# jeun-990806/pim-jpeg-decoder

Measured on AMD Instinct MI355X. Metric: MPixels/sec JPEG->RGB (bit-exact BMP), higher is better.
Workload: dtype int16/int32 (integer IDCT), u8 out

## Files before the change

### pim-jpeg-decoder_amd/csrc/pjd_device_common.h

```cpp
#pragma once
#include <hip/hip_runtime.h>
#include <stdint.h>

#include "pjd_internal.h"

static __constant__ uint8_t c_zz[64] = {
     0,  1,  8, 16,  9,  2,  3, 10, 17, 24, 32, 25, 18, 11,  4,  5,
    12, 19, 26, 33, 40, 48, 41, 34, 27, 20, 13,  6,  7, 14, 21, 28,
    35, 42, 49, 56, 57, 50, 43, 36, 29, 22, 15, 23, 30, 37, 44, 51,
    38, 59, 52, 45, 38, 31, 39, 46, 53, 60, 61, 54, 47, 55, 62, 63
};

__device__ __forceinline__ int pjd_mul_i24(int a, int k)
{
    int r;
    asm("v_mul_i32_i24 %0, %1, %2" : "=v"(r) : "s"(k), "v"(a));
    return r;
}

__device__ __forceinline__ void pjd_idct8(int x0, int x1, int x2, int x3, int x4, int x5, int x6, int x7, int *o)
{
    const int g0 = pjd_mul_i24(x0, 181) >> 5, g1 = pjd_mul_i24(x4, 181) >> 5;
    const int g2 = pjd_mul_i24(x2, 59) >> 3,  g3 = pjd_mul_i24(x6, 49) >> 4;
    const int g4 = pjd_mul_i24(x5, 71) >> 4,  g5 = pjd_mul_i24(x1, 251) >> 5;
    const int g6 = pjd_mul_i24(x7, 25) >> 4,  g7 = pjd_mul_i24(x3, 213) >> 5;
    const int f4 = g4 - g7, f5 = g5 + g6, f6 = g5 - g6, f7 = g4 + g7;
    const int e2 = g2 - g3, e3 = g2 + g3, e5 = f5 - f7, e7 = f5 + f7, e8 = f4 + f6;
    const int d2 = pjd_mul_i24(e2, 181) >> 7, d4 = pjd_mul_i24(f4, 277) >> 8, d5 = pjd_mul_i24(e5, 181) >> 7;
    const int d6 = pjd_mul_i24(f6, 669) >> 8, d8 = pjd_mul_i24(e8, 49) >> 6;
    const int c0 = g0 + g1, c1 = g0 - g1, c2 = d2 - e3, c4 = d4 + d8;
    const int c5 = d5 + e7, c6 = d6 - d8, c8 = c5 - c6;
    const int b0 = c0 + e3, b1 = c1 + c2, b2 = c1 - c2, b3 = c0 - e3, b4 = c4 - c8, b6 = c6 - e7;
    o[0] = (b0 + e7) >> 4; o[1] = (b1 + b6) >> 4; o[2] = (b2 + c8) >> 4; o[3] = (b3 + b4) >> 4;
    o[4] = (b3 - b4) >> 4; o[5] = (b2 - c8) >> 4; o[6] = (b1 - b6) >> 4; o[7] = (b0 - e7) >> 4;
}

__device__ __forceinline__ int pjd_clamp255(int v)
{
    int r;
    asm("v_med3_i32 %0, %1, 0, %2" : "=v"(r) : "v"(v), "s"(255));
    return r;
}

__device__ __forceinline__ void pjd_ycc_to_rgb(int y, int cb, int cr, int &r, int &g, int &b)
{
    r = pjd_clamp255(y + (__mul24(5880414, cr) >> 22) + 128);
    g = pjd_clamp255(y - (__mul24(1442840, cb) >> 22) - (__mul24(2994733, cr) >> 22) + 128);
    b = pjd_clamp255(y + (__mul24(7432306, cb) >> 22) + 128);
}

__device__ __forceinline__ uint32_t pjd_mul_u24(uint32_t a, uint32_t b)
{
    uint32_t r;
    asm("v_mul_u32_u24 %0, %1, %2" : "=v"(r) : "v"(a), "v"(b));
    return r;
}
__device__ __forceinline__ uint32_t pjd_mad_u24(uint32_t a, uint32_t b, uint32_t c)
{
    uint32_t r;
    asm("v_mad_u32_u24 %0, %1, %2, %3" : "=v"(r) : "v"(a), "v"(b), "v"(c));
    return r;
}

__device__ __forceinline__ int pjd_dequant(int coef, unsigned q) { return (int)(int16_t)__mul24(coef, (int)q); }
```

### pim-jpeg-decoder_amd/csrc/pjd_k_backend.hip

```cpp
#include <cstdlib>

#include "pjd_device_common.h"
#include "pjd_kernels.h"

#define TILE_STRIDE 72

__global__ __launch_bounds__(128) void pjd_k_dpu_payload(const uint32_t *__restrict__ meta_all, int16_t *__restrict__ mcus_all)
{
    __shared__ __attribute__((aligned(16))) int16_t tile[12][TILE_STRIDE];
    const int dpu = blockIdx.x / 25, blk = blockIdx.x % 25;
    const uint32_t *m = meta_all + (size_t)dpu * 276;
    int16_t *base = mcus_all + (size_t)dpu * 19200 + blk * 768;
    const int tid = threadIdx.x;
    const int ncomp = (int)m[4];
    const int V = (int)(m[5] & 255), H = (int)(m[6] & 255);

    if (tid < 96) {
        const int du = tid >> 3, r = tid & 7, comp = du >> 2;
        const int4 raw = *reinterpret_cast<const int4 *>(base + du * 64 + r * 8);
        const int16_t *rv = reinterpret_cast<const int16_t *>(&raw);
        int x[8], o[8];
#pragma unroll
        for (int j = 0; j < 8; j++) x[j] = rv[j];
        if (comp < ncomp) {
// ... 261 lines not shown
            if (Y >= height) continue;
            const int16_t *yp = &tile[d0 + lrow + (px0 >> 3)][yoff + (px0 & 7)];
            const uint2 yraw = *reinterpret_cast<const uint2 *>(yp);
            const int y0 = (int16_t)(yraw.x & 0xffff), y1 = (int16_t)(yraw.x >> 16), y2 = (int16_t)(yraw.y & 0xffff), y3 = (int16_t)(yraw.y >> 16);
            const uint32_t q = cy * 8 + (px0 >> hs_log);
            int cf[4], cg[4], cl[4];
            const int n_chroma = hs == 2 ? 2 : 4;
            uint2 cbw = make_uint2(0, 0), crw = make_uint2(0, 0);
            if (nc > 1) { if (hs == 2) cbw.x = *reinterpret_cast<const uint32_t *>(&tile[d0 + nl][q]); else cbw = *reinterpret_cast<const uint2 *>(&tile[d0 + nl][q]); }
            if (nc > 2) { if (hs == 2) crw.x = *reinterpret_cast<const uint32_t *>(&tile[d0 + nl + 1][q]); else crw = *reinterpret_cast<const uint2 *>(&tile[d0 + nl + 1][q]); }
#pragma unroll
            for (int j = 0; j < 4; j++) {
                if (j < n_chroma) {
                    const uint32_t bw = j < 2 ? cbw.x : cbw.y, rw = j < 2 ? crw.x : crw.y;
                    const int cbv = (j & 1) ? (int)(int16_t)(bw >> 16) : (int)(int16_t)(bw & 0xffff);
                    const int crv = (j & 1) ? (int)(int16_t)(rw >> 16) : (int)(int16_t)(rw & 0xffff);
                    const int rC = (__mul24(5880414, crv) >> 22) + 128, bC = (__mul24(7432306, cbv) >> 22) + 128;
                    cg[j] = 128 - (__mul24(1442840, cbv) >> 22) - (__mul24(2994733, crv) >> 22);
                    cf[j] = bmp ? bC : rC;
                    cl[j] = bmp ? rC : bC;
                }
            }
            const int s1 = hs == 2 ? 0 : 1, s2 = hs == 2 ? 1 : 2, s3 = hs == 2 ? 1 : 3;
            const int cf1 = s1 ? cf[1] : cf[0], cg1 = s1 ? cg[1] : cg[0], cl1 = s1 ? cl[1] : cl[0];
            const int cf2 = s2 == 2 ? cf[2] : cf[1], cg2 = s2 == 2 ? cg[2] : cg[1], cl2 = s2 == 2 ? cl[2] : cl[1];
            const int cf3 = s3 == 3 ? cf[3] : cf[1], cg3 = s3 == 3 ? cg[3] : cg[1], cl3 = s3 == 3 ? cl[3] : cl[1];
            const uint32_t f0 = pjd_clamp255(y0 + cf[0]), g0 = pjd_clamp255(y0 + cg[0]), l0 = pjd_clamp255(y0 + cl[0]);
            const uint32_t f1 = pjd_clamp255(y1 + cf1), g1 = pjd_clamp255(y1 + cg1), l1 = pjd_clamp255(y1 + cl1);
            const uint32_t f2 = pjd_clamp255(y2 + cf2), g2 = pjd_clamp255(y2 + cg2), l2 = pjd_clamp255(y2 + cl2);
            const uint32_t f3 = pjd_clamp255(y3 + cf3), g3 = pjd_clamp255(y3 + cg3), l3 = pjd_clamp255(y3 + cl3);
            if (PLANAR) {
                const size_t plane = (size_t)stride * height;
                uint8_t *o = out + (size_t)Y * stride + X;
                if (X + 4 <= width) {
                    reinterpret_cast<PjdPx4 *>(o)->a = f0 | (f1 << 8) | (f2 << 16) | (f3 << 24);
                    reinterpret_cast<PjdPx4 *>(o + plane)->a = g0 | (g1 << 8) | (g2 << 16) | (g3 << 24);
                    reinterpret_cast<PjdPx4 *>(o + 2 * plane)->a = l0 | (l1 << 8) | (l2 << 16) | (l3 << 24);
                } else {
                    o[0] = (uint8_t)f0; o[plane] = (uint8_t)g0; o[2 * plane] = (uint8_t)l0;
                    if (X + 1 < width) { o[1] = (uint8_t)f1; o[plane + 1] = (uint8_t)g1; o[2 * plane + 1] = (uint8_t)l1; }
                    if (X + 2 < width) { o[2] = (uint8_t)f2; o[plane + 2] = (uint8_t)g2; o[2 * plane + 2] = (uint8_t)l2; }
                }
                continue;
            }
            uint8_t *o = bmp ? out + 26 + (size_t)(height - 1 - Y) * stride + X * 3
                             : out + (size_t)Y * stride + X * 3;
            if (X + 4 <= width) {
                Px12 v;
                v.a = f0 | (g0 << 8) | (l0 << 16) | (f1 << 24);
                v.b = g1 | (l1 << 8) | (f2 << 16) | (g2 << 24);
                v.c = l2 | (f3 << 8) | (g3 << 16) | (l3 << 24);
                *reinterpret_cast<Px12 *>(o) = v;
            } else {
                o[0] = (uint8_t)f0; o[1] = (uint8_t)g0; o[2] = (uint8_t)l0;
                if (X + 1 < width) { o[3] = (uint8_t)f1; o[4] = (uint8_t)g1; o[5] = (uint8_t)l1; }
                if (X + 2 < width) { o[6] = (uint8_t)f2; o[7] = (uint8_t)g2; o[8] = (uint8_t)l2; }
            }
        }
    }
}

struct __attribute__((packed)) PjdPx12 { uint32_t a, b, c; };

template <int HS, int VS, bool BMP, bool PLANAR = false>
__device__ __forceinline__ void pjd_colour_store(const int16_t (*tile)[TILE_STRIDE], const uint32_t *mcu_xy, uint8_t *out,
                                                 uint32_t width, uint32_t height, uint32_t stride, uint32_t ncomp,
                                                 uint32_t n_mcu, uint32_t tid, size_t plane = 0)
{
    static_assert(!(BMP && PLANAR), "a BMP file image is interleaved");
    constexpr uint32_t MW = 8 * HS, MH = 8 * VS, NL = HS * VS;
    constexpr uint32_t CG_LOG = HS == 2 ? 2 : 1;
    constexpr int NCH = 4 / HS;
    const uint32_t dus = NL + ncomp - 1;
    const uint32_t per_row = n_mcu << CG_LOG;
    const uint32_t lane = tid & 63, wv = tid >> 6;
    for (uint32_t rg = wv; rg < 8; rg += PJD_IDCT_THREADS / 64) {
        for (uint32_t idx = lane; idx < per_row; idx += 64) {
            const uint32_t ml = idx >> CG_LOG, px0 = (idx & ((1u << CG_LOG) - 1)) * 4;
            const uint32_t xy = mcu_xy[ml];
            const uint32_t X = __umul24(xy & 0xffffu, MW) + px0, Y0 = __umul24(xy >> 16, MH) + rg * VS;
            if (X >= width || Y0 >= height) continue;
            const uint32_t d0 = __umul24(ml, dus);
            int cf[NCH], cg[NCH], cl[NCH];
            {
                const uint32_t q = rg * 8 + px0 / HS;
                uint32_t cbw[2] = {0, 0}, crw[2] = {0, 0};
                if (ncomp > 1) {
                    if (HS == 2) cbw[0] = *reinterpret_cast<const uint32_t *>(&tile[d0 + NL][q]);
                    else { const uint2 t = *reinterpret_cast<const uint2 *>(&tile[d0 + NL][q]); cbw[0] = t.x; cbw[1] = t.y; }
                }
                if (ncomp > 2) {
                    if (HS == 2) crw[0] = *reinterpret_cast<const uint32_t *>(&tile[d0 + NL + 1][q]);
                    else { const uint2 t = *reinterpret_cast<const uint2 *>(&tile[d0 + NL + 1][q]); crw[0] = t.x; crw[1] = t.y; }
                }
#pragma unroll
                for (int j = 0; j < NCH; j++) {
                    const uint32_t bw = cbw[j >> 1], rw = crw[j >> 1];
                    const int cbv = (j & 1) ? (int)bw >> 16 : (int)(int16_t)(bw & 0xffff);
                    const int crv = (j & 1) ? (int)rw >> 16 : (int)(int16_t)(rw & 0xffff);
                    const int rC = (__mul24(5880414, crv) >> 22) + 128, bC = (__mul24(7432306, cbv) >> 22) + 128;
                    cg[j] = 128 - (__mul24(1442840, cbv) >> 22) - (__mul24(2994733, crv) >> 22);
                    cf[j] = BMP ? bC : rC;
                    cl[j] = BMP ? rC : bC;
                }
            }
#pragma unroll
            for (int v = 0; v < VS; v++) {
                const uint32_t Y = Y0 + v;
                if (Y >= height) break;
                const uint32_t py = rg * VS + v;
                const int16_t *yp = &tile[d0 + (py >> 3) * HS + (px0 >> 3)][(py & 7) * 8 + (px0 & 7)];
                const uint2 yraw = *reinterpret_cast<const uint2 *>(yp);
                const int y0 = (int16_t)(yraw.x & 0xffff), y1 = (int)yraw.x >> 16, y2 = (int16_t)(yraw.y & 0xffff), y3 = (int)yraw.y >> 16;
                constexpr int s1 = HS == 2 ? 0 : 1, s2 = HS == 2 ? 1 : 2, s3 = HS == 2 ? 1 : 3;
                const uint32_t f0 = pjd_clamp255(y0 + cf[0]), g0 = pjd_clamp255(y0 + cg[0]), l0 = pjd_clamp255(y0 + cl[0]);
                const uint32_t f1 = pjd_clamp255(y1 + cf[s1]), g1 = pjd_clamp255(y1 + cg[s1]), l1 = pjd_clamp255(y1 + cl[s1]);
                const uint32_t f2 = pjd_clamp255(y2 + cf[s2]), g2 = pjd_clamp255(y2 + cg[s2]), l2 = pjd_clamp255(y2 + cl[s2]);
                const uint32_t f3 = pjd_clamp255(y3 + cf[s3]), g3 = pjd_clamp255(y3 + cg[s3]), l3 = pjd_clamp255(y3 + cl[s3]);
                if (PLANAR) {
                    uint8_t *o = out + (size_t)Y * stride + X;
                    if (X + 4 <= width) {
                        reinterpret_cast<PjdPx4 *>(o)->a = f0 | (f1 << 8) | (f2 << 16) | (f3 << 24);
                        reinterpret_cast<PjdPx4 *>(o + plane)->a = g0 | (g1 << 8) | (g2 << 16) | (g3 << 24);
                        reinterpret_cast<PjdPx4 *>(o + 2 * plane)->a = l0 | (l1 << 8) | (l2 << 16) | (l3 << 24);
                    } else {
                        o[0] = (uint8_t)f0; o[plane] = (uint8_t)g0; o[2 * plane] = (uint8_t)l0;
                        if (X + 1 < width) { o[1] = (uint8_t)f1; o[plane + 1] = (uint8_t)g1; o[2 * plane + 1] = (uint8_t)l1; }
                        if (X + 2 < width) { o[2] = (uint8_t)f2; o[plane + 2] = (uint8_t)g2; o[2 * plane + 2] = (uint8_t)l2; }
                    }
                    continue;
                }
                uint8_t *o = BMP ? out + 26 + (size_t)(height - 1 - Y) * stride + X * 3 : out + (size_t)Y * stride + X * 3;
                if (X + 4 <= width) {
                    PjdPx12 px;
                    px.a = f0 | (g0 << 8) | (l0 << 16) | (f1 << 24);
                    px.b = g1 | (l1 << 8) | (f2 << 16) | (g2 << 24);
                    px.c = l2 | (f3 << 8) | (g3 << 16) | (l3 << 24);
                    *reinterpret_cast<PjdPx12 *>(o) = px;
                } else {
                    o[0] = (uint8_t)f0; o[1] = (uint8_t)g0; o[2] = (uint8_t)l0;
                    if (X + 1 < width) { o[3] = (uint8_t)f1; o[4] = (uint8_t)g1; o[5] = (uint8_t)l1; }
                    if (X + 2 < width) { o[6] = (uint8_t)f2; o[7] = (uint8_t)g2; o[8] = (uint8_t)l2; }
                }
            }
        }
    }
}

__device__ __forceinline__ void pjd_bmp_header(uint8_t *out, uint32_t width, uint32_t height, uint32_t stride, uint32_t tid)
{
    if (tid >= 26) return;
    const uint32_t size = 26 + height * stride;
    uint8_t hb = 0;
    switch (tid) {
        case 0: hb = 'B'; break;  case 1: hb = 'M'; break;
        case 2: hb = size & 255; break; case 3: hb = (size >> 8) & 255; break;
        case 4: hb = (size >> 16) & 255; break; case 5: hb = (size >> 24) & 255; break;
        case 10: hb = 0x1A; break; case 14: hb = 12; break;
        case 18: hb = width & 255; break; case 19: hb = (width >> 8) & 255; break;
        case 20: hb = height & 255; break; case 21: hb = (height >> 8) & 255; break;
        case 22: hb = 1; break; case 24: hb = 24; break;
        default: hb = 0;
    }
    out[tid] = hb;
}

template <int HS, int VS, bool BMP, int S, bool PLANAR = false>
__device__ __forceinline__ void pjd_colour_store_scaled(const int16_t (*tile)[TILE_STRIDE], const uint32_t *mcu_xy, uint8_t *out,
                                                        uint32_t width, uint32_t height, uint32_t stride, uint32_t ncomp,
                                                        uint32_t n_mcu, uint32_t tid)
{
    static_assert(!(BMP && PLANAR), "a BMP file image is interleaved");
    constexpr uint32_t MW = 8 * HS, MH = 8 * VS, NL = HS * VS;
    constexpr uint32_t CG_LOG = HS == 2 ? 2 : 1;
    constexpr uint32_t S_LOG = S == 2 ? 1 : (S == 4 ? 2 : 3);
    constexpr uint32_t BR_LOG = (VS == 2 ? 4 : 3) - S_LOG;
    constexpr int NCH = 4 / HS;
    constexpr int NO = S < 4 ? 4 / S : 1;
    constexpr int PX_LOG = S < 4 ? S_LOG : 2;
    static_assert(MH % S == 0 && S % VS == 0, "a box lies inside one MCU and covers whole chroma rows");
    const uint32_t dus = NL + ncomp - 1;
    const uint32_t tasks = n_mcu << (CG_LOG + BR_LOG);
    const uint32_t sh = (height + S - 1) >> S_LOG;
    for (uint32_t t = tid; t < tasks; t += PJD_IDCT_THREADS) {
        const uint32_t ml = t >> (CG_LOG + BR_LOG), j = (t >> CG_LOG) & ((1u << BR_LOG) - 1), px0 = (t & ((1u << CG_LOG) - 1)) * 4;
        const uint32_t xy = mcu_xy[ml];
        const uint32_t X = __umul24(xy & 0xffffu, MW) + px0, Yb = __umul24(xy >> 16, MH) + j * S;
// ... 117 lines not shown

template <bool SCALED, bool PLANAR = false>
__device__ __forceinline__ void pjd_colour_dispatch(const int16_t (*tile)[TILE_STRIDE], const uint32_t *mcu_xy, const PjdDevBatch &B,
                                                    const PjdDevImage &im, const PjdDevIdctWg &wg, uint32_t tid)
{
    if (SCALED && (im.flags & PJD_IF_SCALE_MASK)) { pjd_colour_dispatch_scaled<PLANAR>(tile, mcu_xy, B, im, wg, tid); return; }
    uint8_t *out = B.out + im.out_off;
    const uint32_t width = im.width, height = im.height, stride = im.out_stride, nc = im.ncomp, n = wg.n_mcu;
    if (PLANAR) {
        const size_t plane = (size_t)stride * height;
        switch ((im.hs - 1) | ((im.vs - 1) << 1)) {
            case 0: pjd_colour_store<1, 1, false, true>(tile, mcu_xy, out, width, height, stride, nc, n, tid, plane); break;
            case 1: pjd_colour_store<2, 1, false, true>(tile, mcu_xy, out, width, height, stride, nc, n, tid, plane); break;
            case 2: pjd_colour_store<1, 2, false, true>(tile, mcu_xy, out, width, height, stride, nc, n, tid, plane); break;
            default: pjd_colour_store<2, 2, false, true>(tile, mcu_xy, out, width, height, stride, nc, n, tid, plane); break;
        }
        return;
    }
    const bool bmp = (im.flags & PJD_IF_BMP) != 0;
    if (bmp && wg.first_mcu == 0) pjd_bmp_header(out, width, height, stride, tid);
    const uint32_t mode = (im.hs - 1) | ((im.vs - 1) << 1) | (bmp ? 4u : 0u);
    switch (mode) {
        case 0: pjd_colour_store<1, 1, false>(tile, mcu_xy, out, width, height, stride, nc, n, tid); break;
        case 1: pjd_colour_store<2, 1, false>(tile, mcu_xy, out, width, height, stride, nc, n, tid); break;
        case 2: pjd_colour_store<1, 2, false>(tile, mcu_xy, out, width, height, stride, nc, n, tid); break;
        case 3: pjd_colour_store<2, 2, false>(tile, mcu_xy, out, width, height, stride, nc, n, tid); break;
        case 4: pjd_colour_store<1, 1, true>(tile, mcu_xy, out, width, height, stride, nc, n, tid); break;
        case 5: pjd_colour_store<2, 1, true>(tile, mcu_xy, out, width, height, stride, nc, n, tid); break;
        case 6: pjd_colour_store<1, 2, true>(tile, mcu_xy, out, width, height, stride, nc, n, tid); break;
        default: pjd_colour_store<2, 2, true>(tile, mcu_xy, out, width, height, stride, nc, n, tid); break;
    }
}

template <bool SCALED>
__global__ __launch_bounds__(PJD_IDCT_THREADS) void pjd_k_idct_colour(PjdDevBatch B, const PjdDevIdctWg *__restrict__ wgs, const uint64_t *__restrict__ dense_base)
{
#define PJD_DENSE_PLANAR false
#include "pjd_k_idct_dense_body.h"
#undef PJD_DENSE_PLANAR
}

template <bool SCALED>
__global__ __launch_bounds__(PJD_IDCT_THREADS) void pjd_k_idct_colour_planar(PjdDevBatch B, const PjdDevIdctWg *__restrict__ wgs, const uint64_t *__restrict__ dense_base)
{
#define PJD_DENSE_PLANAR true
#include "pjd_k_idct_dense_body.h"
#undef PJD_DENSE_PLANAR
}


#define PJD_DPP_STEP(OP, v, ctrl, rmask)                                                               \
    do { const uint32_t t_ = (uint32_t)__builtin_amdgcn_update_dpp(0, (int)(v), ctrl, rmask, 0xf, false); v = OP(v, t_); } while (0)
__device__ __forceinline__ uint32_t pjd_op_add(uint32_t a, uint32_t b) { return a + b; }
__device__ __forceinline__ uint32_t pjd_op_max(uint32_t a, uint32_t b) { return a > b ? a : b; }
__device__ __forceinline__ uint32_t pjd_op_pkadd(uint32_t a, uint32_t b)
{
    typedef unsigned short u16x2 __attribute__((ext_vector_type(2)));
    return __builtin_bit_cast(uint32_t, (u16x2)(__builtin_bit_cast(u16x2, a) + __builtin_bit_cast(u16x2, b)));
}
__device__ __forceinline__ uint32_t pjd_op_pksub(uint32_t a, uint32_t b)
{
    typedef unsigned short u16x2 __attribute__((ext_vector_type(2)));
    return __builtin_bit_cast(uint32_t, (u16x2)(__builtin_bit_cast(u16x2, a) - __builtin_bit_cast(u16x2, b)));
}
#define PJD_WAVE_SCAN(OP, v)                                                                           \
    do {                                                                                                \
        PJD_DPP_STEP(OP, v, 0x111, 0xf); PJD_DPP_STEP(OP, v, 0x112, 0xf); PJD_DPP_STEP(OP, v, 0x114, 0xf);  \
        PJD_DPP_STEP(OP, v, 0x118, 0xf); PJD_DPP_STEP(OP, v, 0x142, 0xa); PJD_DPP_STEP(OP, v, 0x143, 0xc);  \
    } while (0)
__device__ __forceinline__ uint32_t pjd_wave_prev(uint32_t v)
{
    const uint32_t r = (uint32_t)__builtin_amdgcn_update_dpp(0, (int)v, 0x138 , 0xf, 0xf, false);
    return r;
}

__device__ __forceinline__ void pjd_tile_put(uint32_t tile_lds, uint32_t u, uint32_t pos, uint32_t v)
{
    const uint32_t a = pjd_mad_u24(u, TILE_STRIDE * 2u, tile_lds + 2u * pos);
    *reinterpret_cast<__attribute__((address_space(3))) int16_t *>(a) = (int16_t)v;
}

template <bool SCALED, bool PLANAR = false>
__device__ __forceinline__ void pjd_idct_range(const PjdDevBatch &B, uint32_t iwg, int16_t (*tile)[TILE_STRIDE], uint32_t (*qz)[64], uint32_t *mcu_xy,
                                               uint8_t *comp_of, uint32_t *wagg, uint32_t *ltab)
{
    const PjdDevIdctWg wg = B.iwgs[iwg];
    const PjdDevImage &im = B.images[wg.image];
    if ((im.flags & PJD_IF_SEQUENTIAL) || (B.status[wg.image] & PJD_STW_NEEDS_EXACT)) return;
    const uint32_t tid = threadIdx.x, lane = tid & 63, wv = tid >> 6;
    const uint32_t dus = im.dus_per_mcu, nl = im.n_luma;
    const uint32_t n_du = wg.n_mcu * dus;
    const uint32_t RI = im.restart_interval;

    const bool quirk = !(im.flags & PJD_IF_STANDARD_ZIGZAG);
    if (tid < 192) {
        const uint32_t nat = (!quirk && (tid & 63) == 48) ? 58u : c_zz[tid & 63];
        uint32_t v = (uint32_t)B.qtab[(size_t)wg.image * 192 + (tid & ~63u) + nat] | (nat << 16);
        if (quirk && (tid & 63) == 52) v = 1u | (64u << 16);
        qz[tid >> 6][tid & 63] = v;
    }
    static_assert(TILE_STRIDE == 72, "the padding cell of a tile row is element 64");
    for (uint32_t i = tid; i < n_du * (TILE_STRIDE * 2 / 16); i += PJD_IDCT_THREADS)
        reinterpret_cast<uint4 *>(&tile[0][0])[i] = make_uint4(i % 9u == 8u ? (uint32_t)(uint16_t)PJD_COEF_SENTINEL : 0u, 0, 0, 0);
    if (tid < PJD_IDCT_MAX_DU) {
        const uint32_t kk = tid % dus;
        comp_of[tid] = (uint8_t)(kk < nl ? 0 : kk - nl + 1);
    }

    const unsigned long long err_key = B.imstate[wg.image].err_key;
    const uint32_t n_valid = pjd_units_decoded(err_key, wg.first_mcu * dus, n_du);
    const uint32_t err_byte = (uint32_t)(err_key >> 35);
    const PjdDevMark mark = B.marks[iwg];
    const uint32_t lane_end = im.lane_base + im.n_lane;
    uint32_t q = mark.lane, n = mark.ent_off;
    (void)n;
    if (n_valid == 0) { q = im.lane_base; n = 0; }
    else if (q < im.lane_base || q >= lane_end) return;
    uint32_t pred0[3];
    {
        const PjdDevLaneDc ld = B.lane_dc[q];
        const uint16_t *carry = B.dc_blk + (size_t)(q / PJD_DC_BLOCK) * 8 + 4;
#pragma unroll
        for (int c = 0; c < 3; c++) pred0[c] = (uint32_t)ld.dc_in[c] + (ld.abs ? 0u : (uint32_t)carry[c]) + mark.acc[c];
    }
    __syncthreads();
#if defined(PJD_IDCT_STOP_AFTER) && PJD_IDCT_STOP_AFTER == 0
    if (tile[0][0] == 12345) B.out[0] = 1;
    return;
#endif
    {
        const uint32_t U0 = wg.first_mcu * dus;
        const uint32_t tile_lds = (uint32_t)(uintptr_t)(__attribute__((address_space(3))) int16_t *)&tile[0][0];
        const uint32_t g0 = mark.ent_off / PJD_GROUP;
        uint32_t q_end = 0xffffffffu, g_end = 0;
        if (n_valid == n_du && iwg + 1 < im.iwg_base + im.n_iwg) {
            const PjdDevMark nm = B.marks[iwg + 1];
            if (nm.lane >= q && nm.lane < lane_end) { q_end = nm.lane; g_end = nm.ent_off / PJD_GROUP; }
        }
        for (uint32_t qw = q; n_valid != 0; qw += 32) {
            bool more = false;
            if (tid < 32) {
                const uint32_t ql = qw + tid;
                uint32_t ng = 0, fd = 0, ne = 0;
                if (ql < lane_end) {
                    const PjdDevLaneInfo li = B.lane_info[ql];
                    fd = (li.first_du & 0x0fffffffu) - U0;
                    ne = li.n_ent;
                    const bool in = (ql == q || (int)fd < (int)n_valid) && (ql == q || B.lanes[ql].byte_start <= err_byte);
                    if (in && ql <= q_end) {
                        const uint32_t gs = ql == q ? g0 : 0u, all = (ne + PJD_GROUP - 1) / PJD_GROUP;
                        uint32_t ge = ql == q_end ? (g_end + 1 < all ? g_end + 1 : all) : all;
                        ng = ge > gs ? ge - gs : 0u;
                    }
                    more = in && ql < q_end;
                }
                uint32_t inc = ng;
#pragma unroll
                for (int off = 1; off < 32; off <<= 1) { const uint32_t t = __shfl_up(inc, off); if ((int)tid >= off) inc += t; }
                ltab[tid] = inc - ng; ltab[32 + tid] = fd; ltab[64 + tid] = ne;
                if (tid == 31) { wagg[0] = inc; wagg[1] = more ? 1u : 0u; }
            }
            __syncthreads();
            const uint32_t G = wagg[0];
            const bool again = wagg[1] != 0 && qw + 32 < lane_end;
            for (uint32_t w = tid; w < G; w += PJD_IDCT_THREADS) {
                uint32_t li_ = 0;
#pragma unroll
                for (uint32_t step = 16; step != 0; step >>= 1) if (ltab[li_ + step] <= w) li_ += step;
                const uint32_t ql = qw + li_;
                const uint32_t g = w - ltab[li_] + (ql == q ? g0 : 0u);
                const uint32_t ne = ltab[64 + li_];
                const uint32_t cnt = ne - g * PJD_GROUP < PJD_GROUP ? ne - g * PJD_GROUP : PJD_GROUP;
                const uint4 *src = reinterpret_cast<const uint4 *>(B.ent + im.ent_base + (size_t)(ql - im.lane_base) * im.lane_cap + (size_t)g * PJD_GROUP);
                const uint4 r0 = src[0], r1 = src[1];
                const uint32_t wds[8] = {r0.x, r0.y, r0.z, r0.w, r1.x, r1.y, r1.z, r1.w};
                const uint32_t head = wds[0];
                uint32_t u = ltab[32 + li_] + (head >> 8);
                uint32_t slot = head & 63u;
#pragma unroll
                for (int k = 1; k < PJD_GROUP / 2; k++) {
                    const uint32_t sw = wds[k];
                    const bool on = (uint32_t)(2 * k) < cnt;
                    {
                        const bool dc = slot == 0;
                        const uint32_t f = dc ? 1u : sw & 31u;
                        const uint32_t ns = slot + f, pos = ns - 1u;
                        if (on && f != 0 && pos < 64 && u < n_valid) {
                            const int val = dc ? (int)(int16_t)(sw & 0xffffu) : (int)(sw << 16) >> 21;
                            const uint32_t qe = qz[comp_of[u]][pos];
                            pjd_tile_put(tile_lds, u, qe >> 16, pjd_mul_u24((uint32_t)val, qe));
                        }
                        if (on) {
                            const bool last = f == 0 || ns > 63;
                            slot = last ? 0u : ns;
                            u += last ? 1u : 0u;
                        }
                    }
                    {
                        const uint32_t f = (sw >> 16) & 31u;
                        const bool onb = on && f <= 16;
                        const uint32_t pos = slot + f - 1u;
                        if (onb && f != 0 && pos < 64 && u < n_valid) {
                            const int val = (int)sw >> 21;
                            const uint32_t qe = qz[comp_of[u]][pos];
                            pjd_tile_put(tile_lds, u, qe >> 16, pjd_mul_u24((uint32_t)val, qe));
                        }
                        if (onb) {
                            const uint32_t ns = slot + f;
                            const bool last = f == 0 || ns > 63;
                            slot = last ? 0u : ns;
                            u += last ? 1u : 0u;
                        }
                    }
                }
            }
            __syncthreads();
            if (!again) break;
        }
    }
#if defined(PJD_IDCT_STOP_AFTER) && PJD_IDCT_STOP_AFTER == 1
    if (tile[0][0] == 12345) B.out[0] = 1;
    return;
#endif
    if (wv != 0) {
        for (uint32_t i = tid - 64; i < n_du * 7; i += PJD_IDCT_THREADS - 64) {
            const uint32_t u = i / 7, r = 1 + (i - u * 7);
            if (r == 4 && tile[u][64] != (int16_t)PJD_COEF_SENTINEL) tile[u][38] = (int16_t)pjd_dequant((int)tile[u][64], qz[comp_of[u]][48] & 0xffffu);
            pjd_tile_row(tile, u, r);
        }
    } else {
        const uint32_t d0 = wg.first_mcu * dus;
        const uint32_t q0y = qz[0][0] & 0xffffu, q0b = qz[1][0] & 0xffffu, q0r = qz[2][0] & 0xffffu;
        uint32_t cy = (pred0[0] * q0y) & 0xffffu, cc = ((pred0[1] * q0b) & 0xffffu) | ((pred0[2] * q0r) << 16);
        for (uint32_t base = 0; base < n_du; base += 64) {
            const uint32_t u = base + lane;
            const bool on = u < n_valid;
            const uint32_t d = d0 + u, m = d / dus, kk = d - m * dus, comp = kk < nl ? 0 : kk - nl + 1;
            const uint32_t dv = on ? (uint32_t)(uint16_t)tile[on ? u : 0][0] : 0u;
            const bool head = on && kk == 0 && (m == im.first_mcu || (RI != 0 && m % RI == 0));
            uint32_t vy = comp == 0 ? dv : 0u, vc = comp == 1 ? dv : (comp == 2 ? dv << 16 : 0u);
            PJD_WAVE_SCAN(pjd_op_add, vy);
            PJD_WAVE_SCAN(pjd_op_pkadd, vc);
            uint32_t hpos = head ? lane + 1 : 0u;
            PJD_WAVE_SCAN(pjd_op_max, hpos);
            const uint32_t hl = hpos ? hpos - 1 : 0u;
            const uint32_t by = __shfl(vy, (int)hl) - __shfl(comp == 0 ? dv : 0u, (int)hl);
            const uint32_t bc = __shfl(vc, (int)hl), bc_own = __shfl(comp == 1 ? dv : (comp == 2 ? dv << 16 : 0u), (int)hl);
            uint32_t ty = vy, tc = vc;
            if (hpos) { ty -= by; tc = pjd_op_pksub(tc, pjd_op_pksub(bc, bc_own)); }
            else { ty += cy; tc = pjd_op_pkadd(tc, cc); }
            if (on) {
                const uint32_t dcv = comp == 0 ? ty : (comp == 1 ? tc : tc >> 16);
                tile[u][0] = (int16_t)dcv;
            }
            cy = __shfl(ty, 63); cc = __shfl(tc, 63);
        }
    }
    if (tid < wg.n_mcu) {
        const uint32_t m = wg.first_mcu + tid, my = m / im.mcux;
        mcu_xy[tid] = (my << 16) | (m - my * im.mcux);
    }
    __syncthreads();
#if defined(PJD_IDCT_STOP_AFTER) && PJD_IDCT_STOP_AFTER == 2
    if (tile[0][0] == 12345) B.out[0] = 1;
    return;
#endif
    for (uint32_t u = tid; u < n_du; u += PJD_IDCT_THREADS) pjd_tile_row(tile, u, 0);
    __syncthreads();
    for (uint32_t i = tid; i < n_du * 8; i += PJD_IDCT_THREADS) pjd_tile_col(tile, i >> 3, i & 7);
    __syncthreads();
#if defined(PJD_IDCT_STOP_AFTER) && PJD_IDCT_STOP_AFTER == 3
    if (tile[0][0] == 12345) B.out[0] = 1;
    return;
#endif
    pjd_colour_dispatch<SCALED, PLANAR>(tile, mcu_xy, B, im, wg, tid);
}

__global__ __launch_bounds__(PJD_IDCT_THREADS) void pjd_k_idct_colour_lanes(PjdDevBatch B, const uint32_t *__restrict__ order, int sweep)
{
    __shared__ __attribute__((aligned(16))) int16_t tile[PJD_IDCT_MAX_DU][TILE_STRIDE];
    __shared__ uint32_t qz[3][64];
    __shared__ uint32_t mcu_xy[PJD_IDCT_MAX_DU];
    __shared__ uint8_t comp_of[PJD_IDCT_MAX_DU];
    __shared__ uint32_t wagg[2];
    __shared__ uint32_t ltab[96];

#if PJD_IDCT_PRIO
    __builtin_amdgcn_s_setprio(PJD_IDCT_PRIO);
#endif
    const uint32_t iwg = order ? order[blockIdx.x] : blockIdx.x;
    if (sweep && __hip_atomic_load(B.range_done + iwg, __ATOMIC_RELAXED, __HIP_MEMORY_SCOPE_AGENT)) return;
    pjd_idct_range<false>(B, iwg, tile, qz, mcu_xy, comp_of, wagg, ltab);
}

__global__ __launch_bounds__(PJD_IDCT_THREADS) void pjd_k_idct_colour_lanes_scaled(PjdDevBatch B, const uint32_t *__restrict__ order)
{
    __shared__ __attribute__((aligned(16))) int16_t tile[PJD_IDCT_MAX_DU][TILE_STRIDE];
    __shared__ uint32_t qz[3][64];
    __shared__ uint32_t mcu_xy[PJD_IDCT_MAX_DU];
    __shared__ uint8_t comp_of[PJD_IDCT_MAX_DU];
    __shared__ uint32_t wagg[2];
    __shared__ uint32_t ltab[96];

#if PJD_IDCT_PRIO
    __builtin_amdgcn_s_setprio(PJD_IDCT_PRIO);
#endif
    pjd_idct_range<true>(B, order ? order[blockIdx.x] : blockIdx.x, tile, qz, mcu_xy, comp_of, wagg, ltab);
}

template <bool SCALED>
__global__ __launch_bounds__(PJD_IDCT_THREADS) void pjd_k_idct_colour_lanes_planar(PjdDevBatch B, const uint32_t *__restrict__ order)
{
    __shared__ __attribute__((aligned(16))) int16_t tile[PJD_IDCT_MAX_DU][TILE_STRIDE];
    __shared__ uint32_t qz[3][64];
    __shared__ uint32_t mcu_xy[PJD_IDCT_MAX_DU];
    __shared__ uint8_t comp_of[PJD_IDCT_MAX_DU];
    __shared__ uint32_t wagg[2];
    __shared__ uint32_t ltab[96];

#if PJD_IDCT_PRIO
    __builtin_amdgcn_s_setprio(PJD_IDCT_PRIO);
#endif
    pjd_idct_range<SCALED, true>(B, order ? order[blockIdx.x] : blockIdx.x, tile, qz, mcu_xy, comp_of, wagg, ltab);
}

__global__ __launch_bounds__(PJD_IDCT_THREADS) void pjd_k_idct_pull(PjdDevBatch B)
{
    __shared__ __attribute__((aligned(16))) int16_t tile[PJD_IDCT_MAX_DU][TILE_STRIDE];
    __shared__ uint32_t qz[3][64];
    __shared__ uint32_t mcu_xy[PJD_IDCT_MAX_DU];
    __shared__ uint8_t comp_of[PJD_IDCT_MAX_DU];
    __shared__ uint32_t wagg[2];
    __shared__ uint32_t ltab[96];
    if (threadIdx.x == 0) {
        uint32_t started = 0;
        for (uint32_t it = 0; it < 64 && !started; it++) {
            started = __hip_atomic_load(B.ticket, __ATOMIC_RELAXED, __HIP_MEMORY_SCOPE_AGENT) >= B.n_hwg ? 1u : 0u;
            if (!started) __builtin_amdgcn_s_sleep(64);
        }
        wagg[1] = started;
    }
    __syncthreads();
    if (wagg[1] == 0) return;
    for (uint32_t slot = blockIdx.x; slot < B.n_iwg; slot += gridDim.x) {
        __syncthreads();
        if (threadIdx.x == 0) {
            uint32_t v = 0;
            for (uint32_t it = 0; it < PJD_PULL_SPIN_LIMIT; it++) {
                v = __hip_atomic_load(B.ready_list + slot, __ATOMIC_RELAXED, __HIP_MEMORY_SCOPE_AGENT);
                if (v) break;
                __builtin_amdgcn_s_sleep(64);
            }
            wagg[0] = v;
        }
        __syncthreads();
        const uint32_t v = wagg[0];
        __syncthreads();
        if (v == 0) return;
#if defined(PJD_PULL_EXPERIMENT) && PJD_PULL_EXPERIMENT == 1
        continue;
#endif
        __atomic_thread_fence(__ATOMIC_ACQUIRE);
        pjd_idct_range<false>(B, v - 1, tile, qz, mcu_xy, comp_of, wagg, ltab);
        __syncthreads();
        if (threadIdx.x == 0) __hip_atomic_store(B.range_done + (v - 1), 1u, __ATOMIC_RELAXED, __HIP_MEMORY_SCOPE_AGENT);
    }
}

void pjd_launch_idct_colour_lanes(hipStream_t s, const PjdDevBatch &b, bool scaled, bool planar)
{
    if (b.n_iwg == 0) return;
    if (planar && scaled) hipLaunchKernelGGL(pjd_k_idct_colour_lanes_planar<true>, dim3(b.n_iwg), dim3(PJD_IDCT_THREADS), 0, s, b, (const uint32_t *)nullptr);
    else if (planar) hipLaunchKernelGGL(pjd_k_idct_colour_lanes_planar<false>, dim3(b.n_iwg), dim3(PJD_IDCT_THREADS), 0, s, b, (const uint32_t *)nullptr);
    else if (scaled) hipLaunchKernelGGL(pjd_k_idct_colour_lanes_scaled, dim3(b.n_iwg), dim3(PJD_IDCT_THREADS), 0, s, b, (const uint32_t *)nullptr);
    else hipLaunchKernelGGL(pjd_k_idct_colour_lanes, dim3(b.n_iwg), dim3(PJD_IDCT_THREADS), 0, s, b, (const uint32_t *)nullptr, 0);
}

void pjd_launch_idct_pull(hipStream_t s, const PjdDevBatch &b)
{
    static const uint32_t workers = [] { const char *e = std::getenv("PJD_PULL_WORKERS"); const int v = e ? std::atoi(e) : 0; return (uint32_t)(v > 0 ? v : 512); }();
    const uint32_t n = b.n_iwg < workers ? b.n_iwg : workers;
    if (n) hipLaunchKernelGGL(pjd_k_idct_pull, dim3(n), dim3(PJD_IDCT_THREADS), 0, s, b);
}

void pjd_launch_idct_sweep(hipStream_t s, const PjdDevBatch &b)
{
    if (b.n_iwg) hipLaunchKernelGGL(pjd_k_idct_colour_lanes, dim3(b.n_iwg), dim3(PJD_IDCT_THREADS), 0, s, b, (const uint32_t *)nullptr, 1);
}

void pjd_launch_group_idct(hipStream_t s, const PjdDevBatch &b, const PjdDevGroup &g, bool scaled, bool planar)
{
    if (!g.iwg_count) return;
    if (planar && scaled) hipLaunchKernelGGL(pjd_k_idct_colour_lanes_planar<true>, dim3(g.iwg_count), dim3(PJD_IDCT_THREADS), 0, s, b, (const uint32_t *)(b.iwg_order + g.iwg_first));
    else if (planar) hipLaunchKernelGGL(pjd_k_idct_colour_lanes_planar<false>, dim3(g.iwg_count), dim3(PJD_IDCT_THREADS), 0, s, b, (const uint32_t *)(b.iwg_order + g.iwg_first));
    else if (scaled) hipLaunchKernelGGL(pjd_k_idct_colour_lanes_scaled, dim3(g.iwg_count), dim3(PJD_IDCT_THREADS), 0, s, b, (const uint32_t *)(b.iwg_order + g.iwg_first));
    else hipLaunchKernelGGL(pjd_k_idct_colour_lanes, dim3(g.iwg_count), dim3(PJD_IDCT_THREADS), 0, s, b, b.iwg_order + g.iwg_first, 0);
}

__global__ __launch_bounds__(PJD_DC_BLOCK) void pjd_k_group_dc(PjdDevBatch B, const uint32_t *__restrict__ images)
{
    __shared__ uint32_t sy[PJD_DC_BLOCK], scb[PJD_DC_BLOCK], scr[PJD_DC_BLOCK], sf[PJD_DC_BLOCK];
    const uint32_t i = images[blockIdx.x], tid = threadIdx.x;
    const PjdDevImage &im = B.images[i];
    if (tid == 0) {
        const int32_t st = B.status[i];
        if (!(st & PJD_STW_NEEDS_EXACT)) {
            const PjdDevImState s = B.imstate[i];
            const bool has_err = s.err_key != ~0ull;
            const uint32_t err_pos = (uint32_t)(s.err_key >> 32);
            if (s.flag_pos != 0xffffffffu && (!has_err || s.flag_pos <= err_pos)) B.status[i] = st | PJD_STW_NEEDS_EXACT;
            else if (has_err) B.status[i] = (int32_t)((s.err_key >> 1) & 7u);
        }
    }
    uint32_t cy = 0, ccb = 0, ccr = 0;
    for (uint32_t base = 0; base < im.n_lane; base += PJD_DC_BLOCK) {
        const uint32_t q = im.lane_base + base + tid;
        const bool on = base + tid < im.n_lane;
        uint32_t vy = 0, vcb = 0, vcr = 0, head = 0;
        if (on) {
            const PjdDevLaneInfo li = B.lane_info[q];
            vy = li.dc_sum[0]; vcb = li.dc_sum[1]; vcr = li.dc_sum[2]; head = li.first_du >> 31;
        }
        sy[tid] = vy; scb[tid] = vcb; scr[tid] = vcr; sf[tid] = head;
        __syncthreads();
        for (uint32_t off = 1; off < PJD_DC_BLOCK; off <<= 1) {
            uint32_t ay = 0, acb = 0, acr = 0, af = 0;
            const bool take = tid >= off;
            if (take) { ay = sy[tid - off]; acb = scb[tid - off]; acr = scr[tid - off]; af = sf[tid - off]; }
            const uint32_t myf = sf[tid];
            __syncthreads();
            if (take) {
                if (!myf) { sy[tid] += ay; scb[tid] += acb; scr[tid] += acr; }
                sf[tid] = myf | af;
            }
            __syncthreads();
        }
        if (on) {
            PjdDevLaneDc d;
            d.dc_in[0] = d.dc_in[1] = d.dc_in[2] = 0;
            d.abs = 1;
            if (!head) {
                uint32_t py = cy, pcb = ccb, pcr = ccr;
                if (tid > 0) {
                    const bool h = sf[tid - 1] != 0;
                    py = (h ? 0u : cy) + sy[tid - 1]; pcb = (h ? 0u : ccb) + scb[tid - 1]; pcr = (h ? 0u : ccr) + scr[tid - 1];
                }
// ... 34 lines not shown
```

Measured before the change: 131,700.

## Add packed int16 colour-conversion fast path and precompute DC-scan metadata in shared memory

Adds a fast colour-conversion path that uses packed 16-bit saturating adds and v_sat_pk_u8_i16 to produce four pixels per step. It is taken when the chroma values are within a safe range and the whole 4-pixel group lies inside the image width, replacing per-pixel med3 clamps and byte packing. Separately, it replaces integer division/modulo by small constants with reciprocal multiplies, and restricts tile zeroing to the coefficient cells plus one sentinel store per data unit. It also precomputes per-DU component and restart-head flags in shared memory so the DC prediction scan no longer divides per lane. This adds a shared array and a branch on chroma range, and the packed path relies on int16 saturation matching the old clamps.

```diff
diff --git a/pim-jpeg-decoder_amd/csrc/pjd_device_common.h b/pim-jpeg-decoder_amd/csrc/pjd_device_common.h
--- a/pim-jpeg-decoder_amd/csrc/pjd_device_common.h
+++ b/pim-jpeg-decoder_amd/csrc/pjd_device_common.h
@@ -49,6 +49,35 @@
     b = pjd_clamp255(y + (__mul24(7432306, cb) >> 22) + 128);
 }
 
+__device__ __forceinline__ uint32_t pjd_pk_add_i16_sat(uint32_t a, uint32_t b)
+{
+    uint32_t r;
+    asm("v_pk_add_i16 %0, %1, %2 clamp" : "=v"(r) : "v"(a), "v"(b));
+    return r;
+}
+__device__ __forceinline__ uint32_t pjd_pk_add_u16(uint32_t a, uint32_t b)
+{
+    uint32_t r;
+    asm("v_pk_add_u16 %0, %1, %2" : "=v"(r) : "v"(a), "v"(b));
+    return r;
+}
+__device__ __forceinline__ uint32_t pjd_sat_pk_u8_i16(uint32_t a)
+{
+    uint32_t r;
+    asm("v_sat_pk_u8_i16 %0, %1" : "=v"(r) : "v"(a));
+    return r;
+}
+__device__ __forceinline__ void pjd_sat_pk_u8_i16_hi(uint32_t &d, uint32_t a)
+{
+    asm("v_sat_pk_u8_i16_sdwa %0, %1 dst_sel:WORD_1 dst_unused:UNUSED_PRESERVE src0_sel:DWORD" : "+v"(d) : "v"(a));
+}
+__device__ __forceinline__ uint32_t pjd_pack_i16(int lo, int hi)
+{
+    return __builtin_amdgcn_perm((uint32_t)hi, (uint32_t)lo, 0x05040100u);
+}
+__device__ __forceinline__ uint32_t pjd_perm(uint32_t hi, uint32_t lo, uint32_t sel) { return __builtin_amdgcn_perm(hi, lo, sel); }
+__device__ __forceinline__ uint32_t pjd_chroma_out_of_range(uint32_t w) { return pjd_pk_add_u16(w, 0x40004000u) & 0x80008000u; }
+
 __device__ __forceinline__ uint32_t pjd_mul_u24(uint32_t a, uint32_t b)
 {
     uint32_t r;
@@ -62,4 +91,7 @@
     return r;
 }
 
+static __constant__ uint32_t c_recip16[11] = {0, 65536, 32768, 21846, 16384, 13108, 10923, 9363, 8192, 7282, 6554};
+__device__ __forceinline__ uint32_t pjd_div_small(uint32_t u, uint32_t recip16) { return pjd_mul_u24(u, recip16) >> 16; }
+
 __device__ __forceinline__ int pjd_dequant(int coef, unsigned q) { return (int)(int16_t)__mul24(coef, (int)q); }
diff --git a/pim-jpeg-decoder_amd/csrc/pjd_k_backend.hip b/pim-jpeg-decoder_amd/csrc/pjd_k_backend.hip
--- a/pim-jpeg-decoder_amd/csrc/pjd_k_backend.hip
+++ b/pim-jpeg-decoder_amd/csrc/pjd_k_backend.hip
@@ -367,6 +367,7 @@
             if (X >= width || Y0 >= height) continue;
             const uint32_t d0 = __umul24(ml, dus);
             int cf[NCH], cg[NCH], cl[NCH];
+            bool fast = X + 4 <= width;
             {
                 const uint32_t q = rg * 8 + px0 / HS;
                 uint32_t cbw[2] = {0, 0}, crw[2] = {0, 0};
@@ -378,6 +379,9 @@
                     if (HS == 2) crw[0] = *reinterpret_cast<const uint32_t *>(&tile[d0 + NL + 1][q]);
                     else { const uint2 t = *reinterpret_cast<const uint2 *>(&tile[d0 + NL + 1][q]); crw[0] = t.x; crw[1] = t.y; }
                 }
+                uint32_t oor = pjd_chroma_out_of_range(cbw[0]) | pjd_chroma_out_of_range(crw[0]);
+                if (HS == 1) oor |= pjd_chroma_out_of_range(cbw[1]) | pjd_chroma_out_of_range(crw[1]);
+                fast = fast && oor == 0;
 #pragma unroll
                 for (int j = 0; j < NCH; j++) {
                     const uint32_t bw = cbw[j >> 1], rw = crw[j >> 1];
@@ -388,6 +392,41 @@
                     cf[j] = BMP ? bC : rC;
                     cl[j] = BMP ? rC : bC;
                 }
+            }
+            if (fast) {
+                constexpr int s1 = HS == 2 ? 0 : 1, s2 = HS == 2 ? 1 : 2, s3 = HS == 2 ? 1 : 3;
+                const uint32_t pf01 = pjd_pack_i16(cf[0], cf[s1]), pf23 = pjd_pack_i16(cf[s2], cf[s3]);
+                const uint32_t pg01 = pjd_pack_i16(cg[0], cg[s1]), pg23 = pjd_pack_i16(cg[s2], cg[s3]);
+                const uint32_t pl01 = pjd_pack_i16(cl[0], cl[s1]), pl23 = pjd_pack_i16(cl[s2], cl[s3]);
+#pragma unroll
+                for (int v = 0; v < VS; v++) {
+                    const uint32_t Y = Y0 + v;
+                    if (Y >= height) break;
+                    const uint32_t py = rg * VS + v;
+                    const int16_t *yp = &tile[d0 + (py >> 3) * HS + (px0 >> 3)][(py & 7) * 8 + (px0 & 7)];
+                    const uint2 yraw = *reinterpret_cast<const uint2 *>(yp);
+                    const uint32_t f01 = pjd_pk_add_i16_sat(yraw.x, pf01), f23 = pjd_pk_add_i16_sat(yraw.y, pf23);
+                    const uint32_t g01 = pjd_pk_add_i16_sat(yraw.x, pg01), g23 = pjd_pk_add_i16_sat(yraw.y, pg23);
+                    const uint32_t l01 = pjd_pk_add_i16_sat(yraw.x, pl01), l23 = pjd_pk_add_i16_sat(yraw.y, pl23);
+                    if (PLANAR) {
+                        uint32_t f = pjd_sat_pk_u8_i16(f01), g = pjd_sat_pk_u8_i16(g01), l = pjd_sat_pk_u8_i16(l01);
+                        pjd_sat_pk_u8_i16_hi(f, f23); pjd_sat_pk_u8_i16_hi(g, g23); pjd_sat_pk_u8_i16_hi(l, l23);
+                        uint8_t *o = out + (size_t)Y * stride + X;
+                        reinterpret_cast<PjdPx4 *>(o)->a = f;
+                        reinterpret_cast<PjdPx4 *>(o + plane)->a = g;
+                        reinterpret_cast<PjdPx4 *>(o + 2 * plane)->a = l;
+                    } else {
+                        uint32_t p = pjd_sat_pk_u8_i16(f01), m = pjd_sat_pk_u8_i16(g01), r = pjd_sat_pk_u8_i16(f23);
+                        pjd_sat_pk_u8_i16_hi(p, l01); pjd_sat_pk_u8_i16_hi(m, g23); pjd_sat_pk_u8_i16_hi(r, l23);
+                        PjdPx12 px;
+                        px.a = pjd_perm(m, p, 0x01020400u);
+                        px.b = pjd_perm(m, pjd_perm(p, r, 0x00000700u), 0x06020105u);
+                        px.c = pjd_perm(m, r, 0x03070102u);
+                        uint8_t *o = BMP ? out + 26 + (size_t)(height - 1 - Y) * stride + X * 3 : out + (size_t)Y * stride + X * 3;
+                        *reinterpret_cast<PjdPx12 *>(o) = px;
+                    }
+                }
+                continue;
             }
 #pragma unroll
             for (int v = 0; v < VS; v++) {
@@ -671,7 +710,7 @@
 
 template <bool SCALED, bool PLANAR = false>
 __device__ __forceinline__ void pjd_idct_range(const PjdDevBatch &B, uint32_t iwg, int16_t (*tile)[TILE_STRIDE], uint32_t (*qz)[64], uint32_t *mcu_xy,
-                                               uint8_t *comp_of, uint32_t *wagg, uint32_t *ltab)
+                                               uint8_t *comp_of, uint8_t *du_head, uint32_t *wagg, uint32_t *ltab)
 {
     const PjdDevIdctWg wg = B.iwgs[iwg];
     const PjdDevImage &im = B.images[wg.image];
@@ -689,11 +728,18 @@
         qz[tid >> 6][tid & 63] = v;
     }
     static_assert(TILE_STRIDE == 72, "the padding cell of a tile row is element 64");
-    for (uint32_t i = tid; i < n_du * (TILE_STRIDE * 2 / 16); i += PJD_IDCT_THREADS)
-        reinterpret_cast<uint4 *>(&tile[0][0])[i] = make_uint4(i % 9u == 8u ? (uint32_t)(uint16_t)PJD_COEF_SENTINEL : 0u, 0, 0, 0);
+    for (uint32_t i = tid; i < n_du * 8; i += PJD_IDCT_THREADS)
+        *reinterpret_cast<uint4 *>(&tile[i >> 3][(i & 7) * 8]) = make_uint4(0, 0, 0, 0);
+    if (tid < n_du) *reinterpret_cast<uint4 *>(&tile[tid][64]) = make_uint4((uint32_t)(uint16_t)PJD_COEF_SENTINEL, 0, 0, 0);
     if (tid < PJD_IDCT_MAX_DU) {
-        const uint32_t kk = tid % dus;
+        const uint32_t ml = pjd_div_small(tid, c_recip16[dus]), kk = tid - __umul24(ml, dus);
         comp_of[tid] = (uint8_t)(kk < nl ? 0 : kk - nl + 1);
+        if (kk != 0) du_head[tid] = 0;
+    }
+    if (tid < wg.n_mcu) {
+        const uint32_t m = wg.first_mcu + tid, my = m / im.mcux;
+        mcu_xy[tid] = (my << 16) | (m - my * im.mcux);
+        du_head[__umul24(tid, dus)] = (uint8_t)(m == im.first_mcu || (RI != 0 && m % RI == 0));
     }
 
     const unsigned long long err_key = B.imstate[wg.image].err_key;
@@ -813,20 +859,19 @@
 #endif
     if (wv != 0) {
         for (uint32_t i = tid - 64; i < n_du * 7; i += PJD_IDCT_THREADS - 64) {
-            const uint32_t u = i / 7, r = 1 + (i - u * 7);
+            const uint32_t u = pjd_div_small(i, c_recip16[7]), r = 1 + (i - __umul24(u, 7u));
             if (r == 4 && tile[u][64] != (int16_t)PJD_COEF_SENTINEL) tile[u][38] = (int16_t)pjd_dequant((int)tile[u][64], qz[comp_of[u]][48] & 0xffffu);
             pjd_tile_row(tile, u, r);
         }
     } else {
-        const uint32_t d0 = wg.first_mcu * dus;
         const uint32_t q0y = qz[0][0] & 0xffffu, q0b = qz[1][0] & 0xffffu, q0r = qz[2][0] & 0xffffu;
         uint32_t cy = (pred0[0] * q0y) & 0xffffu, cc = ((pred0[1] * q0b) & 0xffffu) | ((pred0[2] * q0r) << 16);
         for (uint32_t base = 0; base < n_du; base += 64) {
             const uint32_t u = base + lane;
             const bool on = u < n_valid;
-            const uint32_t d = d0 + u, m = d / dus, kk = d - m * dus, comp = kk < nl ? 0 : kk - nl + 1;
-            const uint32_t dv = on ? (uint32_t)(uint16_t)tile[on ? u : 0][0] : 0u;
-            const bool head = on && kk == 0 && (m == im.first_mcu || (RI != 0 && m % RI == 0));
+            const uint32_t us = on ? u : 0u, comp = comp_of[us];
+            const uint32_t dv = on ? (uint32_t)(uint16_t)tile[us][0] : 0u;
+            const bool head = on && du_head[us] != 0;
             uint32_t vy = comp == 0 ? dv : 0u, vc = comp == 1 ? dv : (comp == 2 ? dv << 16 : 0u);
             PJD_WAVE_SCAN(pjd_op_add, vy);
             PJD_WAVE_SCAN(pjd_op_pkadd, vc);
@@ -845,10 +890,6 @@
             cy = __shfl(ty, 63); cc = __shfl(tc, 63);
         }
     }
-    if (tid < wg.n_mcu) {
-        const uint32_t m = wg.first_mcu + tid, my = m / im.mcux;
-        mcu_xy[tid] = (my << 16) | (m - my * im.mcux);
-    }
     __syncthreads();
 #if defined(PJD_IDCT_STOP_AFTER) && PJD_IDCT_STOP_AFTER == 2
     if (tile[0][0] == 12345) B.out[0] = 1;
@@ -871,6 +912,7 @@
     __shared__ uint32_t qz[3][64];
     __shared__ uint32_t mcu_xy[PJD_IDCT_MAX_DU];
     __shared__ uint8_t comp_of[PJD_IDCT_MAX_DU];
+    __shared__ uint8_t du_head[PJD_IDCT_MAX_DU];
     __shared__ uint32_t wagg[2];
     __shared__ uint32_t ltab[96];
 
@@ -879,7 +921,7 @@
 #endif
     const uint32_t iwg = order ? order[blockIdx.x] : blockIdx.x;
     if (sweep && __hip_atomic_load(B.range_done + iwg, __ATOMIC_RELAXED, __HIP_MEMORY_SCOPE_AGENT)) return;
-    pjd_idct_range<false>(B, iwg, tile, qz, mcu_xy, comp_of, wagg, ltab);
+    pjd_idct_range<false>(B, iwg, tile, qz, mcu_xy, comp_of, du_head, wagg, ltab);
 }
 
 __global__ __launch_bounds__(PJD_IDCT_THREADS) void pjd_k_idct_colour_lanes_scaled(PjdDevBatch B, const uint32_t *__restrict__ order)
@@ -888,13 +930,14 @@
     __shared__ uint32_t qz[3][64];
     __shared__ uint32_t mcu_xy[PJD_IDCT_MAX_DU];
     __shared__ uint8_t comp_of[PJD_IDCT_MAX_DU];
+    __shared__ uint8_t du_head[PJD_IDCT_MAX_DU];
     __shared__ uint32_t wagg[2];
     __shared__ uint32_t ltab[96];
 
 #if PJD_IDCT_PRIO
     __builtin_amdgcn_s_setprio(PJD_IDCT_PRIO);
 #endif
-    pjd_idct_range<true>(B, order ? order[blockIdx.x] : blockIdx.x, tile, qz, mcu_xy, comp_of, wagg, ltab);
+    pjd_idct_range<true>(B, order ? order[blockIdx.x] : blockIdx.x, tile, qz, mcu_xy, comp_of, du_head, wagg, ltab);
 }
 
 template <bool SCALED>
@@ -904,13 +947,14 @@
     __shared__ uint32_t qz[3][64];
     __shared__ uint32_t mcu_xy[PJD_IDCT_MAX_DU];
     __shared__ uint8_t comp_of[PJD_IDCT_MAX_DU];
+    __shared__ uint8_t du_head[PJD_IDCT_MAX_DU];
     __shared__ uint32_t wagg[2];
     __shared__ uint32_t ltab[96];
 
 #if PJD_IDCT_PRIO
     __builtin_amdgcn_s_setprio(PJD_IDCT_PRIO);
 #endif
-    pjd_idct_range<SCALED, true>(B, order ? order[blockIdx.x] : blockIdx.x, tile, qz, mcu_xy, comp_of, wagg, ltab);
+    pjd_idct_range<SCALED, true>(B, order ? order[blockIdx.x] : blockIdx.x, tile, qz, mcu_xy, comp_of, du_head, wagg, ltab);
 }
 
 __global__ __launch_bounds__(PJD_IDCT_THREADS) void pjd_k_idct_pull(PjdDevBatch B)
@@ -919,6 +963,7 @@
     __shared__ uint32_t qz[3][64];
     __shared__ uint32_t mcu_xy[PJD_IDCT_MAX_DU];
     __shared__ uint8_t comp_of[PJD_IDCT_MAX_DU];
+    __shared__ uint8_t du_head[PJD_IDCT_MAX_DU];
     __shared__ uint32_t wagg[2];
     __shared__ uint32_t ltab[96];
     if (threadIdx.x == 0) {
@@ -950,7 +995,7 @@
         continue;
 #endif
         __atomic_thread_fence(__ATOMIC_ACQUIRE);
-        pjd_idct_range<false>(B, v - 1, tile, qz, mcu_xy, comp_of, wagg, ltab);
+        pjd_idct_range<false>(B, v - 1, tile, qz, mcu_xy, comp_of, du_head, wagg, ltab);
         __syncthreads();
         if (threadIdx.x == 0) __hip_atomic_store(B.range_done + (v - 1), 1u, __ATOMIC_RELAXED, __HIP_MEMORY_SCOPE_AGENT);
     }
```

Result: faster. 133,200 (median of 6 runs) (+1.1%).
